# C0ldstudy/PointSecGuard

Measured on AMD Instinct MI355X. Metric: attacked rooms/sec (4096 pts, 40 PGD iters), higher is better.
Workload: dtype f32; 1 GPU; NB non-targeted PGD (eps=0.05, alpha=2/255, 40 iters) on PointNet++ SSG sem_seg, batch=8 rooms x 4096 pts x 9 ch per GPU (BASELINE configs[1]); steps_coalesced_per_launch_max=8, device_batch_rooms=64, launches_in_flight_per_gpu=3, weights=tests/golden/pn2_weights.npz (fitted fixture)

## Files before the change

### pointsecguard_amd/csrc/psg_geometry.hip

```cpp
#include "psg_common.h"
#include "psg_sqdist.cuh"

namespace {

using psg::sqdist;
using psg::sumsq3;

typedef float v2f __attribute__((ext_vector_type(2)));

template <int CTRL, int ROW_MASK>
__device__ __forceinline__ unsigned dpp_max_u32(unsigned v)
{
    unsigned o = (unsigned)__builtin_amdgcn_update_dpp((int)v, (int)v, CTRL, ROW_MASK, 0xF, false);
    return o > v ? o : v;
}
__device__ __forceinline__ unsigned row_max_u32(unsigned v)
{
    v = dpp_max_u32<0xB1, 0xF>(v);
    v = dpp_max_u32<0x4E, 0xF>(v);
    v = dpp_max_u32<0x141, 0xF>(v);
    v = dpp_max_u32<0x140, 0xF>(v);
    return v;
}
__device__ __forceinline__ unsigned wave_max_u32(unsigned v)
{
    v = row_max_u32(v);
    v = dpp_max_u32<0x142, 0xA>(v);
    v = dpp_max_u32<0x143, 0xC>(v);
    return (unsigned)__builtin_amdgcn_readlane((int)v, 63);
}

template <int NT, int PPT>
__global__ __launch_bounds__(NT) void fps_kernel(const float *__restrict__ xyz, int n_clouds, int N, int S,
                                                 const int32_t *__restrict__ start, int32_t *__restrict__ out)
{
    constexpr int NW = NT / 64;
    extern __shared__ float smem[];
    float *s_xyz = smem;
    uint2 *s_part = (uint2 *)(smem + NT * PPT * 3);

    const int p = blockIdx.x;
    const int tid = threadIdx.x, lane = tid & 63, wave = tid >> 6;
    const float *src = xyz + (size_t)(p % n_clouds) * N * 3;
    for (int i = tid; i < NT * PPT * 3; i += NT) s_xyz[i] = i < N * 3 ? src[i] : 0.0f;
    __syncthreads();

    constexpr int PP = (PPT + 1) / 2;
    v2f px[PP], py[PP], pz[PP], dist[PP];
#pragma unroll
    for (int q = 0; q < PP; ++q) {
        const int i = tid * PPT + 2 * q, i1 = (2 * q + 1 < PPT) ? i + 1 : i;
        px[q] = v2f{s_xyz[3 * i], s_xyz[3 * i1]};
        py[q] = v2f{s_xyz[3 * i + 1], s_xyz[3 * i1 + 1]};
        pz[q] = v2f{s_xyz[3 * i + 2], s_xyz[3 * i1 + 2]};
        dist[q] = v2f{1e10f, 1e10f};
    }
    int far = start[p];
    int32_t *o = out + (size_t)p * S;
    for (int s = 0; s < S; ++s) {
        if (tid == 0) o[s] = far;
        const float cx = s_xyz[3 * far], cy = s_xyz[3 * far + 1], cz = s_xyz[3 * far + 2];
        const v2f cx2 = {cx, cx}, cy2 = {cy, cy}, cz2 = {cz, cz};
        unsigned best = 0u;
        int bq = 0;
#pragma unroll
        for (int q = 0; q < PP; ++q) {
            const v2f dx = px[q] - cx2, dy = py[q] - cy2, dz = pz[q] - cz2;
            const v2f d = ((dx * dx) + (dy * dy)) + (dz * dz);
            dist[q] = v2f{d[0] < dist[q][0] ? d[0] : dist[q][0], d[1] < dist[q][1] ? d[1] : dist[q][1]};
#pragma unroll
            for (int u = 0; u < 2; ++u) {
                if (2 * q + u >= PPT) break;
                unsigned key = (tid * PPT + 2 * q + u) < N ? __float_as_uint(dist[q][u]) : 0u;
                if (key > best) { best = key; bq = 2 * q + u; }
            }
        }
        const unsigned wmax = wave_max_u32(best);
        const unsigned long long hit = __ballot(best == wmax);
        const int src_lane = __builtin_ctzll(hit);
        int widx = __builtin_amdgcn_readlane(tid * PPT + bq, src_lane);
        if (NW > 1) {
            uint2 *slot = s_part + (s & 1) * NW;
            if (lane == 0) slot[wave] = make_uint2(wmax, (unsigned)widx);
            __syncthreads();
            const uint2 part = slot[lane & (NW - 1)];
            const unsigned gmax = row_max_u32(part.x);
            const unsigned long long hw = __ballot(part.x == gmax) & ((1ull << NW) - 1ull);
            widx = __builtin_amdgcn_readlane((int)part.y, __builtin_ctzll(hw));
        }
        far = widx;
    }
}

__global__ void gather_rows_kernel(const float *__restrict__ pts, int n_clouds, int N, int C,
                                   const int32_t *__restrict__ idx, int S, float *__restrict__ out, int P)
{
    size_t total = (size_t)P * S * C;
    for (size_t t = (size_t)blockIdx.x * blockDim.x + threadIdx.x; t < total; t += (size_t)gridDim.x * blockDim.x) {
        int c = (int)(t % C);
        size_t r = t / C;
        int s = (int)(r % S);
        int p = (int)(r / S);
        out[t] = pts[((size_t)(p % n_clouds) * N + idx[(size_t)p * S + s]) * C + c];
    }
}

constexpr int BQ_THREADS = 1024;
constexpr int BQ_CPB = 128;
constexpr int BQ_UNROLL = 4;

__global__ __launch_bounds__(BQ_THREADS) void ball_query_kernel(const float *__restrict__ xyz, int n_clouds,
                                                                const float *__restrict__ new_xyz, int N, int S,
                                                                float r2, int K, int32_t *__restrict__ out)
{
    extern __shared__ float s_soa[];
    const int NP = (N + 255) & ~255;
    float *s_x = s_soa, *s_y = s_soa + NP, *s_z = s_soa + 2 * NP, *s_q = s_soa + 3 * NP;
    const int p = blockIdx.y;
    const float *src = xyz + (size_t)(p % n_clouds) * N * 3;
    for (int i = threadIdx.x; i < NP; i += BQ_THREADS) {
        float x = 0.f, y = 0.f, z = 0.f, q = INFINITY;
        if (i < N) { x = src[3 * i]; y = src[3 * i + 1]; z = src[3 * i + 2]; q = sumsq3(x, y, z); }
        s_x[i] = x; s_y[i] = y; s_z[i] = z; s_q[i] = q;
    }
    __syncthreads();
    const int lane = threadIdx.x & 63, wave = threadIdx.x >> 6;
    const unsigned long long lt_mask = (1ull << lane) - 1ull;
    const int c_end = min(S, (int)(blockIdx.x + 1) * BQ_CPB);
    for (int c = blockIdx.x * BQ_CPB + wave; c < c_end; c += BQ_THREADS / 64) {
        const float *cp = new_xyz + ((size_t)p * S + c) * 3;
        const float cx = cp[0], cy = cp[1], cz = cp[2];
        const float csq = sumsq3(cx, cy, cz);
        const v2f cx2 = {cx, cx}, cy2 = {cy, cy}, cz2 = {cz, cz}, cs2 = {csq, csq}, m2 = {-2.0f, -2.0f};
        int32_t *o = out + ((size_t)p * S + c) * K;
        int cnt = 0, first = N;
        for (int base = 0; base < N && cnt < K; base += 64 * BQ_UNROLL) {
            bool in[BQ_UNROLL];
#pragma unroll
            for (int u = 0; u < BQ_UNROLL; u += 2) {
                const int j = base + u * 64 + lane;
                const v2f qx = {s_x[j], s_x[j + 64]}, qy = {s_y[j], s_y[j + 64]}, qz = {s_z[j], s_z[j + 64]},
                          qs = {s_q[j], s_q[j + 64]};
                v2f dot = cx2 * qx;
                dot = __builtin_elementwise_fma(cy2, qy, dot);
                dot = __builtin_elementwise_fma(cz2, qz, dot);
                const v2f dd = ((m2 * dot) + cs2) + qs;
                in[u] = !(dd[0] > r2);
                in[u + 1] = !(dd[1] > r2);
            }
#pragma unroll
            for (int u = 0; u < BQ_UNROLL; ++u) {
                unsigned long long m = __ballot(in[u]);
                if (m) {
                    if (cnt == 0) first = base + u * 64 + __builtin_ctzll(m);
                    int pos = cnt + __popcll(m & lt_mask);
                    if (in[u] && pos < K) o[pos] = base + u * 64 + lane;
                    cnt += __popcll(m);
                }
            }
        }
        for (int pos = min(cnt, K) + lane; pos < K; pos += 64) o[pos] = first;
    }
}

constexpr int BQG_CELLS = 4096;
constexpr int BQG_CPB = 1024;

template <int CTRL, int ROW_MASK>
__device__ __forceinline__ unsigned bq_dpp0(unsigned v)
{
    return (unsigned)__builtin_amdgcn_update_dpp(0, (int)v, CTRL, ROW_MASK, 0xF, false);
}
__device__ __forceinline__ unsigned bq_wave_incl_scan(unsigned v)
{
    v += bq_dpp0<0x111, 0xF>(v);
    v += bq_dpp0<0x112, 0xF>(v);
    v += bq_dpp0<0x114, 0xF>(v);
    v += bq_dpp0<0x118, 0xF>(v);
    v += bq_dpp0<0x142, 0xA>(v);
    v += bq_dpp0<0x143, 0xC>(v);
    return v;
}

__global__ __launch_bounds__(BQ_THREADS) void ball_query_grid_kernel(const float *__restrict__ xyz, int n_clouds,
                                                                     const float *__restrict__ new_xyz, int N, int S,
                                                                     float r2, int K, int32_t *__restrict__ out)
{
    extern __shared__ float s_soa[];
    const int NP = (N + 255) & ~255;
    float *s_x = s_soa, *s_y = s_soa + NP, *s_z = s_soa + 2 * NP, *s_q = s_soa + 3 * NP;
    int *s_start = (int *)(s_soa + 4 * NP);
    int *s_cur = s_start + BQG_CELLS + 1;
    unsigned short *s_sorted = (unsigned short *)(s_cur + BQG_CELLS);
    __shared__ float s_red[BQ_THREADS / 64][6];
    __shared__ float s_box[8];
    __shared__ int s_dim[4];
    __shared__ int s_wsum[BQ_THREADS / 64];
    const int tid = threadIdx.x, lane = tid & 63, wave = tid >> 6;
    const int p = blockIdx.y;
    const float *src = xyz + (size_t)(p % n_clouds) * N * 3;
    float mn0 = INFINITY, mn1 = INFINITY, mn2 = INFINITY, mx0 = -INFINITY, mx1 = -INFINITY, mx2 = -INFINITY;
    for (int i = tid; i < NP; i += BQ_THREADS) {
        float x = 0.f, y = 0.f, z = 0.f, q = INFINITY;
        if (i < N) {
            x = src[3 * i]; y = src[3 * i + 1]; z = src[3 * i + 2]; q = sumsq3(x, y, z);
            mn0 = fminf(mn0, x); mn1 = fminf(mn1, y); mn2 = fminf(mn2, z);
            mx0 = fmaxf(mx0, x); mx1 = fmaxf(mx1, y); mx2 = fmaxf(mx2, z);
        }
        s_x[i] = x; s_y[i] = y; s_z[i] = z; s_q[i] = q;
    }
    for (int o = 32; o > 0; o >>= 1) {
        mn0 = fminf(mn0, __shfl_xor(mn0, o)); mn1 = fminf(mn1, __shfl_xor(mn1, o)); mn2 = fminf(mn2, __shfl_xor(mn2, o));
        mx0 = fmaxf(mx0, __shfl_xor(mx0, o)); mx1 = fmaxf(mx1, __shfl_xor(mx1, o)); mx2 = fmaxf(mx2, __shfl_xor(mx2, o));
    }
    if (lane == 0) { s_red[wave][0] = mn0; s_red[wave][1] = mn1; s_red[wave][2] = mn2; s_red[wave][3] = mx0; s_red[wave][4] = mx1; s_red[wave][5] = mx2; }
    __syncthreads();
    if (tid == 0) {
        float lo[3] = {INFINITY, INFINITY, INFINITY}, hi[3] = {-INFINITY, -INFINITY, -INFINITY};
        for (int w = 0; w < BQ_THREADS / 64; ++w)
            for (int a = 0; a < 3; ++a) { lo[a] = fminf(lo[a], s_red[w][a]); hi[a] = fmaxf(hi[a], s_red[w][3 + a]); }
        float maxabs = 0.0f;
        for (int a = 0; a < 3; ++a) maxabs = fmaxf(maxabs, fmaxf(fabsf(lo[a]), fabsf(hi[a])));
        maxabs += sqrtf(r2);
        float edge = 1.05f * sqrtf(r2 + 1e-5f * maxabs * maxabs);
        const bool finite = maxabs < 1e18f;
        int nx, ny, nz;
        for (;;) {
            if (!finite) { nx = ny = nz = 1; edge = 1.0f; break; }
            nx = (int)((hi[0] - lo[0]) / edge) + 1; ny = (int)((hi[1] - lo[1]) / edge) + 1; nz = (int)((hi[2] - lo[2]) / edge) + 1;
            if ((long long)nx * ny * nz <= BQG_CELLS) break;
            edge *= 1.25f;
        }
        s_box[0] = lo[0]; s_box[1] = lo[1]; s_box[2] = lo[2]; s_box[3] = 1.0f / edge;
        s_box[4] = hi[0]; s_box[5] = hi[1]; s_box[6] = hi[2]; s_box[7] = edge;
        s_dim[0] = nx; s_dim[1] = ny; s_dim[2] = nz; s_dim[3] = nx * ny * nz;
    }
    __syncthreads();
    const float bx = s_box[0], by = s_box[1], bz = s_box[2], inv = s_box[3];
    const float hx = s_box[4], hy = s_box[5], hz = s_box[6], edge1 = s_box[7];
    const int nx = s_dim[0], ny = s_dim[1], nz = s_dim[2], ncell = s_dim[3];
    auto cell1 = [&](float v, float b, int n) {
        if (n == 1) return 0;
        const int c = (int)((v - b) * inv);
        return c < 0 ? 0 : (c >= n ? n - 1 : c);
    };
    for (int c = tid; c <= ncell; c += BQ_THREADS) s_start[c] = 0;
    __syncthreads();
    for (int i = tid; i < N; i += BQ_THREADS)
        atomicAdd(&s_start[(cell1(s_z[i], bz, nz) * ny + cell1(s_y[i], by, ny)) * nx + cell1(s_x[i], bx, nx) + 1], 1);
    __syncthreads();
    {
        const int c0 = 1 + 4 * tid;
        int v[4], sum = 0;
#pragma unroll
        for (int u = 0; u < 4; ++u) { v[u] = c0 + u <= ncell ? s_start[c0 + u] : 0; sum += v[u]; v[u] = sum; }
        const int inc = (int)bq_wave_incl_scan((unsigned)sum);
        if (lane == 63) s_wsum[wave] = inc;
        __syncthreads();
        int base = inc - sum;
        for (int w = 0; w < wave; ++w) base += s_wsum[w];
#pragma unroll
        for (int u = 0; u < 4; ++u)
            if (c0 + u <= ncell) s_start[c0 + u] = base + v[u];
    }
    __syncthreads();
    for (int c = tid; c < ncell; c += BQ_THREADS) s_cur[c] = s_start[c];
    __syncthreads();
    for (int i = tid; i < N; i += BQ_THREADS) {
        const int cell = (cell1(s_z[i], bz, nz) * ny + cell1(s_y[i], by, ny)) * nx + cell1(s_x[i], bx, nx);
        s_sorted[atomicAdd(&s_cur[cell], 1)] = (unsigned short)i;
    }
    __syncthreads();
    const int words = NP >> 5;
    unsigned *bm = (unsigned *)s_cur + wave * words;
    const int c_end = min(S, (int)(blockIdx.x + 1) * BQG_CPB);
    for (int c = blockIdx.x * BQG_CPB + wave; c < c_end; c += BQ_THREADS / 64) {
        for (int w = lane; w < words; w += 64) bm[w] = 0u;
        const float *cp = new_xyz + ((size_t)p * S + c) * 3;
        const float cx = cp[0], cy = cp[1], cz = cp[2];
        const float csq = sumsq3(cx, cy, cz);
        const int ix = cell1(cx, bx, nx), iy = cell1(cy, by, ny), iz = cell1(cz, bz, nz);
        int start = 0, len = 0;
        const bool off_cloud = !(cx >= bx - edge1 && cx <= hx + edge1 && cy >= by - edge1 && cy <= hy + edge1 && cz >= bz - edge1 &&
                                 cz <= hz + edge1);
        if (off_cloud) {
            len = lane == 0 ? N : 0;
        } else if (lane < 9) {
            const int z = iz + lane / 3 - 1, y = iy + lane % 3 - 1;
            if (z >= 0 && z < nz && y >= 0 && y < ny) {
                const int x0 = ix > 0 ? ix - 1 : 0, x1 = ix + 1 < nx ? ix + 1 : nx - 1;
                const int lin = (z * ny + y) * nx + x0;
                start = s_start[lin];
                len = s_start[lin + (x1 - x0) + 1] - start;
            }
        }
        const int incl = (int)bq_wave_incl_scan((unsigned)len);
        const int T = __builtin_amdgcn_readlane(incl, 8);
        const int off = incl - len;
        __builtin_amdgcn_fence(__ATOMIC_SEQ_CST, "wavefront");
        __builtin_amdgcn_wave_barrier();
        for (int i0 = 0; i0 < T; i0 += 64) {
            const int i = i0 + lane;
            int pos = -1;
#pragma unroll
            for (int r = 0; r < 9; ++r) {
                const int o = __builtin_amdgcn_readlane(off, r), l = __builtin_amdgcn_readlane(len, r),
                          st = __builtin_amdgcn_readlane(start, r);
                pos = (i >= o && i < o + l) ? st + (i - o) : pos;
            }
            if (pos >= 0) {
                const int j = s_sorted[pos];
                const float dd = sqdist(cx, cy, cz, csq, s_x[j], s_y[j], s_z[j], s_q[j]);
                if (!(dd > r2)) atomicOr(&bm[j >> 5], 1u << (j & 31));
            }
        }
        __builtin_amdgcn_fence(__ATOMIC_SEQ_CST, "wavefront");
        __builtin_amdgcn_wave_barrier();
        int32_t *o = out + ((size_t)p * S + c) * K;
        int cnt = 0, first = N;
        for (int w0 = 0; w0 < words && cnt < K; w0 += 64) {
            unsigned word = w0 + lane < words ? bm[w0 + lane] : 0u;
            const int pc = __popc(word);
            const int inc = (int)bq_wave_incl_scan((unsigned)pc);
            const int tot = __builtin_amdgcn_readlane(inc, 63);
            if (tot == 0) continue;
            if (cnt == 0) {
                const int fl = __builtin_ctzll(__ballot(word != 0u));
                first = (w0 + fl) * 32 + __builtin_ctz((unsigned)__builtin_amdgcn_readlane((int)word, fl));
            }
            int rank = cnt + inc - pc;
            while (word && rank < K) {
                o[rank++] = (w0 + lane) * 32 + __builtin_ctz(word);
                word &= word - 1u;
            }
            cnt += tot;
        }
        for (int pos = min(cnt, K) + lane; pos < K; pos += 64) o[pos] = first;
        __builtin_amdgcn_wave_barrier();
    }
}
constexpr int NN_THREADS = 256;

__global__ __launch_bounds__(NN_THREADS) void three_nn_kernel(const float *__restrict__ xyz1, int n_clouds1,
                                                              const float *__restrict__ xyz2, int N, int S,
                                                              int32_t *__restrict__ idx, float *__restrict__ w)
{
    extern __shared__ float4 s_pair[];
    const int p = blockIdx.y;
    const float *c2 = xyz2 + (size_t)p * S * 3;
    const int S2 = (S + 1) >> 1;
    for (int i = threadIdx.x; i < S2; i += NN_THREADS) {
        const int a = 2 * i, b = 2 * i + 1;
        const float xa = c2[3 * a], ya = c2[3 * a + 1], za = c2[3 * a + 2];
        float xb = 0.f, yb = 0.f, zb = 0.f, sb = INFINITY;
        if (b < S) { xb = c2[3 * b]; yb = c2[3 * b + 1]; zb = c2[3 * b + 2]; sb = sumsq3(xb, yb, zb); }
        s_pair[2 * i] = make_float4(xa, xb, ya, yb);
        s_pair[2 * i + 1] = make_float4(za, zb, sumsq3(xa, ya, za), sb);
    }
    __syncthreads();
    const int i = blockIdx.x * NN_THREADS + threadIdx.x;
    if (i >= N) return;
    const float *fp = xyz1 + ((size_t)(p % n_clouds1) * N + i) * 3;
    const float fx = fp[0], fy = fp[1], fz = fp[2];
    const float fsq = sumsq3(fx, fy, fz);
    const v2f fx2 = {fx, fx}, fy2 = {fy, fy}, fz2 = {fz, fz}, fs2 = {fsq, fsq}, m2 = {-2.0f, -2.0f};
    float d0 = INFINITY, d1 = INFINITY, d2 = INFINITY;
    int i0 = 0, i1 = 0, i2 = 0;
    for (int jj = 0; jj < S2; ++jj) {
        const float4 q0 = s_pair[2 * jj], q1 = s_pair[2 * jj + 1];
        const v2f qx = {q0.x, q0.y}, qy = {q0.z, q0.w}, qz = {q1.x, q1.y}, qs = {q1.z, q1.w};
        v2f dot = fx2 * qx;
        dot = __builtin_elementwise_fma(fy2, qy, dot);
        dot = __builtin_elementwise_fma(fz2, qz, dot);
        const v2f dd = ((m2 * dot) + fs2) + qs;
#pragma unroll
        for (int u = 0; u < 2; ++u) {
            const float d = dd[u];
            const int j = 2 * jj + u;
            if (d < d2) {
                if (d < d1) {
                    d2 = d1; i2 = i1;
                    if (d < d0) { d1 = d0; i1 = i0; d0 = d; i0 = j; }
                    else { d1 = d; i1 = j; }
                } else { d2 = d; i2 = j; }
            }
        }
    }
    float r0 = __fdiv_rn(1.0f, __fadd_rn(d0, 1e-8f));
    float r1 = __fdiv_rn(1.0f, __fadd_rn(d1, 1e-8f));
    float r2 = __fdiv_rn(1.0f, __fadd_rn(d2, 1e-8f));
    float norm = __fadd_rn(__fadd_rn(r0, r1), r2);
    size_t o = ((size_t)p * N + i) * 3;
    idx[o] = i0; idx[o + 1] = i1; idx[o + 2] = i2;
    w[o] = __fdiv_rn(r0, norm); w[o + 1] = __fdiv_rn(r1, norm); w[o + 2] = __fdiv_rn(r2, norm);
}

__global__ void square_distance_kernel(const float *__restrict__ src, const float *__restrict__ dst, int N, int M,
                                       float *__restrict__ out)
{
    const int b = blockIdx.z;
    const int i = blockIdx.y;
    const float *s = src + ((size_t)b * N + i) * 3;
    const float sx = s[0], sy = s[1], sz = s[2];
    const float ssq = sumsq3(sx, sy, sz);
    for (int j = blockIdx.x * blockDim.x + threadIdx.x; j < M; j += gridDim.x * blockDim.x) {
        const float *d = dst + ((size_t)b * M + j) * 3;
        out[((size_t)b * N + i) * M + j] = sqdist(sx, sy, sz, ssq, d[0], d[1], d[2], sumsq3(d[0], d[1], d[2]));
    }
}

template <int NT, int PPT>
int launch_fps(const float *xyz, int n_clouds, int P, int N, int S, const int32_t *start, int32_t *out,
               hipStream_t st)
{
    size_t lds = (size_t)NT * PPT * 3 * 4 + 2 * (NT / 64) * 8;
    if (lds > 48 * 1024) PSG_CHECK_HIP(psg::allow_big_lds((const void *)fps_kernel<NT, PPT>));
    hipLaunchKernelGGL((fps_kernel<NT, PPT>), dim3(P), dim3(NT), lds, st, xyz, n_clouds, N, S, start, out);
    PSG_LAUNCH_CHECK();
    return PSG_OK;
}

}

extern "C" int psg_fps(psg_ctx *ctx, const float *xyz, int n_clouds, int P, int N, int S, const int32_t *start,
                       int32_t *out_idx, psg_stream stream)
{
    PSG_REQUIRE(ctx && xyz && start && out_idx, "psg_fps: null argument");
    PSG_REQUIRE(P > 0 && n_clouds > 0 && N > 0 && S > 0 && S <= N, "psg_fps: bad sizes P=%d N=%d S=%d", P, N, S);
    PSG_REQUIRE(N <= 8192, "psg_fps: N=%d exceeds the LDS-resident limit 8192", N);
    hipStream_t st = (hipStream_t)stream;
    if (N <= 64) return launch_fps<64, 1>(xyz, n_clouds, P, N, S, start, out_idx, st);
    if (N <= 256) return launch_fps<64, 4>(xyz, n_clouds, P, N, S, start, out_idx, st);
    if (N <= 1024) return launch_fps<256, 4>(xyz, n_clouds, P, N, S, start, out_idx, st);
    static const int cfg = psg::env_int("PSG_FPS_CFG", 0);
    if (N <= 4096 && cfg == 1) return launch_fps<1024, 4>(xyz, n_clouds, P, N, S, start, out_idx, st);
    if (N <= 4096 && (cfg == 3 || (cfg == 0 && P >= 256))) return launch_fps<256, 16>(xyz, n_clouds, P, N, S, start, out_idx, st);
    if (N <= 4096) return launch_fps<512, 8>(xyz, n_clouds, P, N, S, start, out_idx, st);
    return launch_fps<1024, 8>(xyz, n_clouds, P, N, S, start, out_idx, st);
}

extern "C" int psg_square_distance(psg_ctx *ctx, const float *src, const float *dst, int B, int N, int M, float *out,
                                   psg_stream stream)
{
    PSG_REQUIRE(ctx && src && dst && out, "psg_square_distance: null argument");
    PSG_REQUIRE(B > 0 && N > 0 && M > 0 && N <= 65535 && B <= 65535, "psg_square_distance: bad sizes");
    hipLaunchKernelGGL(square_distance_kernel, dim3(std::min(64, psg::ceil_div(M, 256)), N, B), dim3(256), 0,
                       (hipStream_t)stream, src, dst, N, M, out);
    PSG_LAUNCH_CHECK();
    return PSG_OK;
}

extern "C" int psg_gather_points(psg_ctx *ctx, const float *points, int n_clouds, int P, int N, int C,
                                 const int32_t *idx, int S, float *out, psg_stream stream)
{
    PSG_REQUIRE(ctx && points && idx && out, "psg_gather_points: null argument");
    PSG_REQUIRE(P > 0 && n_clouds > 0 && N > 0 && C > 0 && S > 0, "psg_gather_points: bad sizes");
    size_t total = (size_t)P * S * C;
    int blocks = (int)std::min<size_t>((total + 255) / 256, 4096);
    hipLaunchKernelGGL(gather_rows_kernel, dim3(blocks), dim3(256), 0, (hipStream_t)stream, points, n_clouds, N, C,
                       idx, S, out, P);
    PSG_LAUNCH_CHECK();
    return PSG_OK;
}

extern "C" int psg_ball_query(psg_ctx *ctx, const float *xyz, int n_clouds, const float *new_xyz, int P, int N,
                              int S, float r2, int K, int32_t *out_idx, psg_stream stream)
{
    PSG_REQUIRE(ctx && xyz && new_xyz && out_idx, "psg_ball_query: null argument");
    PSG_REQUIRE(P > 0 && n_clouds > 0 && N > 0 && S > 0 && K > 0, "psg_ball_query: bad sizes");
    PSG_REQUIRE(N <= 8192, "psg_ball_query: N=%d exceeds the LDS-resident limit 8192", N);
    static const bool scan_only = []() { const char *v = psg::env_str("PSG_BALL_QUERY"); return v && std::string(v) == "scan"; }();
    const size_t soa = (size_t)((N + 255) & ~255) * 4 * sizeof(float);
    if (!scan_only && N >= 2048 && N <= 4096 && r2 > 0.0f && r2 < 1e30f) {
        const size_t lds = soa + (size_t)(2 * BQG_CELLS + 1) * 4 + (size_t)((N + 255) & ~255) * 2;
        if (lds > 48 * 1024) PSG_CHECK_HIP(psg::allow_big_lds((const void *)ball_query_grid_kernel));
        hipLaunchKernelGGL(ball_query_grid_kernel, dim3(psg::ceil_div(S, BQG_CPB), P), dim3(BQ_THREADS), lds, (hipStream_t)stream, xyz,
                           n_clouds, new_xyz, N, S, r2, K, out_idx);
        PSG_LAUNCH_CHECK();
        return PSG_OK;
    }
    if (soa > 48 * 1024) PSG_CHECK_HIP(psg::allow_big_lds((const void *)ball_query_kernel));
    hipLaunchKernelGGL(ball_query_kernel, dim3(psg::ceil_div(S, BQ_CPB), P), dim3(BQ_THREADS), soa,
                       (hipStream_t)stream, xyz, n_clouds, new_xyz, N, S, r2, K, out_idx);
    PSG_LAUNCH_CHECK();
    return PSG_OK;
}

extern "C" int psg_three_nn(psg_ctx *ctx, const float *xyz1, int n_clouds1, const float *xyz2, int P, int N, int S,
                            int32_t *out_idx, float *out_w, psg_stream stream)
{
    PSG_REQUIRE(ctx && xyz1 && xyz2 && out_idx && out_w, "psg_three_nn: null argument");
    PSG_REQUIRE(P > 0 && n_clouds1 > 0 && N > 0 && S >= 3, "psg_three_nn: bad sizes (need S >= 3)");
    PSG_REQUIRE(S <= 8192, "psg_three_nn: S=%d exceeds the LDS-resident limit 8192", S);
    size_t lds = (size_t)2 * ((S + 1) / 2) * sizeof(float4);
    if (lds > 48 * 1024) PSG_CHECK_HIP(psg::allow_big_lds((const void *)three_nn_kernel));
    hipLaunchKernelGGL(three_nn_kernel, dim3(psg::ceil_div(N, NN_THREADS), P), dim3(NN_THREADS), lds,
                       (hipStream_t)stream, xyz1, n_clouds1, xyz2, N, S, out_idx, out_w);
    PSG_LAUNCH_CHECK();
    return PSG_OK;
}
```

Before: 966.3 rooms/s.

## Restructure FPS argmax with tree max and ballot index recovery, add LDS-free variant

Rewrites the farthest-point-sampling inner loop so distances are kept as unsigned keys, reduced by a ternary max tree, and the winning point index is recovered afterwards with per-slot ballots instead of a serial compare-and-track chain. Adds a template variant that reads coordinates and the selected centroid straight from global memory rather than staging the cloud in LDS, cutting LDS use so more blocks can be resident. Dispatch changes so the 256x16 config uses the LDS-free path for P>256 and the LDS path now needs an explicit env setting. The extra ballots per step and the global centroid loads may add latency. The new path only kicks in for large P, so it may not run for this workload's batch size.

```diff
diff --git a/pointsecguard_amd/csrc/psg_geometry.hip b/pointsecguard_amd/csrc/psg_geometry.hip
--- a/pointsecguard_amd/csrc/psg_geometry.hip
+++ b/pointsecguard_amd/csrc/psg_geometry.hip
@@ -11,7 +11,7 @@
 template <int CTRL, int ROW_MASK>
 __device__ __forceinline__ unsigned dpp_max_u32(unsigned v)
 {
-    unsigned o = (unsigned)__builtin_amdgcn_update_dpp((int)v, (int)v, CTRL, ROW_MASK, 0xF, false);
+    unsigned o = (unsigned)__builtin_amdgcn_update_dpp(0, (int)v, CTRL, ROW_MASK, 0xF, false);
     return o > v ? o : v;
 }
 __device__ __forceinline__ unsigned row_max_u32(unsigned v)
@@ -29,56 +29,88 @@
     v = dpp_max_u32<0x143, 0xC>(v);
     return (unsigned)__builtin_amdgcn_readlane((int)v, 63);
 }
-
-template <int NT, int PPT>
+template <int N>
+__device__ __forceinline__ unsigned max_of(const unsigned (&k)[N])
+{
+    constexpr int G = (N + 2) / 3;
+    unsigned t[G];
+#pragma unroll
+    for (int g = 0; g < G; ++g) {
+        unsigned a = k[3 * g];
+        if (3 * g + 1 < N) a = max(a, k[3 * g + 1]);
+        if (3 * g + 2 < N) a = max(a, k[3 * g + 2]);
+        t[g] = a;
+    }
+    if constexpr (G == 1) return t[0];
+    else return max_of<G>(t);
+}
+
+template <int NT, int PPT, bool LDSC>
 __global__ __launch_bounds__(NT) void fps_kernel(const float *__restrict__ xyz, int n_clouds, int N, int S,
                                                  const int32_t *__restrict__ start, int32_t *__restrict__ out)
 {
     constexpr int NW = NT / 64;
     extern __shared__ float smem[];
     float *s_xyz = smem;
-    uint2 *s_part = (uint2 *)(smem + NT * PPT * 3);
+    uint2 *s_part = (uint2 *)(smem + (LDSC ? NT * PPT * 3 : 0));
 
     const int p = blockIdx.x;
-    const int tid = threadIdx.x, lane = tid & 63, wave = tid >> 6;
+    const int tid = threadIdx.x, lane = tid & 63;
+    const int wave = __builtin_amdgcn_readfirstlane(tid >> 6);
     const float *src = xyz + (size_t)(p % n_clouds) * N * 3;
-    for (int i = tid; i < NT * PPT * 3; i += NT) s_xyz[i] = i < N * 3 ? src[i] : 0.0f;
-    __syncthreads();
+    if (LDSC) {
+        for (int i = tid; i < NT * PPT * 3; i += NT) s_xyz[i] = i < N * 3 ? src[i] : 0.0f;
+        __syncthreads();
+    }
 
     constexpr int PP = (PPT + 1) / 2;
-    v2f px[PP], py[PP], pz[PP], dist[PP];
+    v2f px[PP], py[PP], pz[PP];
+    unsigned dist[PPT];
 #pragma unroll
     for (int q = 0; q < PP; ++q) {
         const int i = tid * PPT + 2 * q, i1 = (2 * q + 1 < PPT) ? i + 1 : i;
-        px[q] = v2f{s_xyz[3 * i], s_xyz[3 * i1]};
-        py[q] = v2f{s_xyz[3 * i + 1], s_xyz[3 * i1 + 1]};
-        pz[q] = v2f{s_xyz[3 * i + 2], s_xyz[3 * i1 + 2]};
-        dist[q] = v2f{1e10f, 1e10f};
-    }
+        if (LDSC) {
+            px[q] = v2f{s_xyz[3 * i], s_xyz[3 * i1]};
+            py[q] = v2f{s_xyz[3 * i + 1], s_xyz[3 * i1 + 1]};
+            pz[q] = v2f{s_xyz[3 * i + 2], s_xyz[3 * i1 + 2]};
+        } else {
+            const bool in0 = i < N, in1 = i1 < N;
+            px[q] = v2f{in0 ? src[3 * i] : 0.0f, in1 ? src[3 * i1] : 0.0f};
+            py[q] = v2f{in0 ? src[3 * i + 1] : 0.0f, in1 ? src[3 * i1 + 1] : 0.0f};
+            pz[q] = v2f{in0 ? src[3 * i + 2] : 0.0f, in1 ? src[3 * i1 + 2] : 0.0f};
+        }
+    }
+#pragma unroll
+    for (int j = 0; j < PPT; ++j) dist[j] = (tid * PPT + j) < N ? __float_as_uint(1e10f) : 0u;
+
     int far = start[p];
     int32_t *o = out + (size_t)p * S;
     for (int s = 0; s < S; ++s) {
         if (tid == 0) o[s] = far;
-        const float cx = s_xyz[3 * far], cy = s_xyz[3 * far + 1], cz = s_xyz[3 * far + 2];
+        float cx, cy, cz;
+        if (LDSC) {
+            cx = s_xyz[3 * far], cy = s_xyz[3 * far + 1], cz = s_xyz[3 * far + 2];
+        } else {
+            const float *c = src + 3 * (size_t)far;
+            cx = c[0], cy = c[1], cz = c[2];
+        }
         const v2f cx2 = {cx, cx}, cy2 = {cy, cy}, cz2 = {cz, cz};
-        unsigned best = 0u;
-        int bq = 0;
 #pragma unroll
         for (int q = 0; q < PP; ++q) {
             const v2f dx = px[q] - cx2, dy = py[q] - cy2, dz = pz[q] - cz2;
             const v2f d = ((dx * dx) + (dy * dy)) + (dz * dz);
-            dist[q] = v2f{d[0] < dist[q][0] ? d[0] : dist[q][0], d[1] < dist[q][1] ? d[1] : dist[q][1]};
-#pragma unroll
-            for (int u = 0; u < 2; ++u) {
-                if (2 * q + u >= PPT) break;
-                unsigned key = (tid * PPT + 2 * q + u) < N ? __float_as_uint(dist[q][u]) : 0u;
-                if (key > best) { best = key; bq = 2 * q + u; }
-            }
-        }
+            dist[2 * q] = min(dist[2 * q], __float_as_uint(d[0]));
+            if (2 * q + 1 < PPT) dist[2 * q + 1] = min(dist[2 * q + 1], __float_as_uint(d[1]));
+        }
+        const unsigned best = max_of<PPT>(dist);
         const unsigned wmax = wave_max_u32(best);
         const unsigned long long hit = __ballot(best == wmax);
         const int src_lane = __builtin_ctzll(hit);
-        int widx = __builtin_amdgcn_readlane(tid * PPT + bq, src_lane);
+        int bq = PPT - 1;
+#pragma unroll
+        for (int j = PPT - 2; j >= 0; --j)
+            if ((__ballot(dist[j] == wmax) >> src_lane) & 1ull) bq = j;
+        int widx = (wave * 64 + src_lane) * PPT + bq;
         if (NW > 1) {
             uint2 *slot = s_part + (s & 1) * NW;
             if (lane == 0) slot[wave] = make_uint2(wmax, (unsigned)widx);
@@ -88,7 +120,7 @@
             const unsigned long long hw = __ballot(part.x == gmax) & ((1ull << NW) - 1ull);
             widx = __builtin_amdgcn_readlane((int)part.y, __builtin_ctzll(hw));
         }
-        far = widx;
+        far = __builtin_amdgcn_readfirstlane(widx);
     }
 }
 
@@ -409,13 +441,13 @@
     }
 }
 
-template <int NT, int PPT>
+template <int NT, int PPT, bool LDSC = true>
 int launch_fps(const float *xyz, int n_clouds, int P, int N, int S, const int32_t *start, int32_t *out,
                hipStream_t st)
 {
-    size_t lds = (size_t)NT * PPT * 3 * 4 + 2 * (NT / 64) * 8;
-    if (lds > 48 * 1024) PSG_CHECK_HIP(psg::allow_big_lds((const void *)fps_kernel<NT, PPT>));
-    hipLaunchKernelGGL((fps_kernel<NT, PPT>), dim3(P), dim3(NT), lds, st, xyz, n_clouds, N, S, start, out);
+    size_t lds = (LDSC ? (size_t)NT * PPT * 3 * 4 : 0) + 2 * (NT / 64) * 8;
+    if (lds > 48 * 1024) PSG_CHECK_HIP(psg::allow_big_lds((const void *)fps_kernel<NT, PPT, LDSC>));
+    hipLaunchKernelGGL((fps_kernel<NT, PPT, LDSC>), dim3(P), dim3(NT), lds, st, xyz, n_clouds, N, S, start, out);
     PSG_LAUNCH_CHECK();
     return PSG_OK;
 }
@@ -434,7 +466,9 @@
     if (N <= 1024) return launch_fps<256, 4>(xyz, n_clouds, P, N, S, start, out_idx, st);
     static const int cfg = psg::env_int("PSG_FPS_CFG", 0);
     if (N <= 4096 && cfg == 1) return launch_fps<1024, 4>(xyz, n_clouds, P, N, S, start, out_idx, st);
-    if (N <= 4096 && (cfg == 3 || (cfg == 0 && P >= 256))) return launch_fps<256, 16>(xyz, n_clouds, P, N, S, start, out_idx, st);
+    if (N <= 4096 && cfg == 3) return launch_fps<256, 16>(xyz, n_clouds, P, N, S, start, out_idx, st);
+    if (N <= 4096 && cfg == 5) return launch_fps<512, 8, false>(xyz, n_clouds, P, N, S, start, out_idx, st);
+    if (N <= 4096 && (cfg == 4 || (cfg == 0 && P > 256))) return launch_fps<256, 16, false>(xyz, n_clouds, P, N, S, start, out_idx, st);
     if (N <= 4096) return launch_fps<512, 8>(xyz, n_clouds, P, N, S, start, out_idx, st);
     return launch_fps<1024, 8>(xyz, n_clouds, P, N, S, start, out_idx, st);
 }
```

Measured after the change: 987.9 rooms/s (median of 6 runs). 1.02x the previous value.
